# Stanford-ILIAD/PantheonRL

Hardware: AMD Instinct MI355X
Metric: env-steps/sec (all agents) Overcooked-simple PPO self-play (higher is better)
Workload: dtype f32; 1 GPU; OvercookedMultiEnv-v0 layout=simple, PPO self-play (two independent PPO learners per GPU), synthetic (n_envs, n_steps, obs_dim) rollouts; n_envs=1024, n_steps=128, obs_dim=62, features=62, n_logits=6, batch_size=32768, n_epochs=10, agents_per_gpu=2, parallelism=2 agent(s) per gpu x1 gpu(s) = 2 learners (single process), launch_mode=graph, gemm_mode=2, action_masks=none, rollout=scripted, rollout_requested=scripted

## Files before the change

pantheonrl_amd/csrc/ph_policy.hip:

```cpp
#include <cstring>
#include <initializer_list>
#include "ph_rowtail.h"
#include "ph_liar_group.h"
#include "ph_pool.h"

namespace ph {


template <int R, int LP, bool VALU>
__device__ __forceinline__ void policy_fwd_body(const FwdArgs& a) {
  extern __shared__ __attribute__((aligned(16))) float smem[];
  constexpr int NT = R * 4;
  const NetDims& nd = a.nd;
  constexpr int Lp = LP, LDO = LP + 1;
  float* bufA = smem;
  float* bufB = bufA + R * LDH;
  float* w1s = bufB + R * LDH;
  float* w2s = w1s + HID * LDH;
  float* wos = w2s + HID * LDH;
  float* outs = wos + HID * LDO;
  float* b1s = outs + R * LDO;
  float* b2s = b1s + HID;
  float* bos = b2s + HID;
  int* rowphys = (int*)(bos + 64);
// ... 120 lines not shown
    return (i == 5 && (tid >> 6) != 1) ? NONE : base + (unsigned)(3 * i) * (unsigned)D * 4u;
  }
  __device__ __forceinline__ static __amdgpu_buffer_rsrc_t block(const float* blk, int n, int D) {
    return __builtin_amdgcn_make_buffer_rsrc(const_cast<float*>(blk), 0, n * D * 4, 0x00020000);
  }
  __device__ __forceinline__ void issue(const float* obs, int n, const NetDims& nd, unsigned base, int tid) {
    const __amdgpu_buffer_rsrc_t rs = block(obs, n, nd.D);
#pragma unroll
    for (int i = 0; i < ITERS; ++i)
      v[i] = __builtin_bit_cast(float, __builtin_amdgcn_raw_buffer_load_b32(rs, slot_offset(base, i, nd.D, tid), 0, 0));
  }
  __device__ __forceinline__ void commit(float* dst, int tid) const {
    const int kk = tid & 63, w = (tid >> 6) - 1;
#pragma unroll
    for (int i = 0; i < ITERS; ++i) {
      const int r = w + 3 * i;
      if (r < 16) dst[r * LDH + kk] = v[i];
    }
  }
  __device__ __forceinline__ void copy_out(float* rb_obs, int n, int D, unsigned base, int tid) const {
    const __amdgpu_buffer_rsrc_t rs = block(rb_obs, n, D);
#pragma unroll
    for (int i = 0; i < ITERS; ++i)
      __builtin_amdgcn_raw_buffer_store_b32(__builtin_bit_cast(unsigned, v[i]), rs, slot_offset(base, i, D, tid), 0, 0);
  }
};

template <int CTRL>
__device__ __forceinline__ float dpp_quad_f(float v) {
  return __builtin_bit_cast(float, __builtin_amdgcn_update_dpp(0, __builtin_bit_cast(int, v), CTRL, 0xF, 0xF, true));
}
__device__ __forceinline__ float quad_sum_f(float v) {
  v += dpp_quad_f<0xB1>(v);
  v += dpp_quad_f<0x4E>(v);
  return v;
}

template <bool KEEP_JOINT>
__device__ __forceinline__ void fwd_args_pin_lean(FwdArgs& a) {
  a.mask = nullptr;
  a.uniforms = nullptr;
  a.given_actions = nullptr;
  a.deterministic = 0;
  a.act_f32 = nullptr;
  a.entropy = nullptr;
  a.logits = nullptr;
#ifndef PH_LEAN_PROF
  a.prof = nullptr;
#endif
  a.pos_env = nullptr;
  a.rec_mask = nullptr;
  if constexpr (!KEEP_JOINT) {
    a.joint = nullptr;
    a.joint_ll = nullptr;
  }
  a.env_mask = nullptr;
  a.host_done = nullptr;
  __builtin_assume(a.rb_obs != nullptr);
  __builtin_assume(a.rb_act != nullptr);
  __builtin_assume(a.rb_rew != nullptr);
  __builtin_assume(a.rb_es != nullptr);
  __builtin_assume(a.rb_val != nullptr);
  __builtin_assume(a.rb_logp != nullptr);
  __builtin_assume(a.es_in != nullptr);
}
bool fwd_args_lean(const FwdArgs& a, bool joint_ok = false) {
  static int enabled = -1;
  if (enabled < 0) {
    const char* e = getenv("PH_ROLLOUT_LEAN");
    enabled = (e && e[0] == '0') ? 0 : 1;
  }
#ifdef PH_LEAN_PROF
  constexpr bool lean_prof = true;
#else
  constexpr bool lean_prof = false;
#endif
  return enabled && !a.mask && !a.uniforms && !a.given_actions && !a.deterministic && !a.act_f32 && !a.entropy && !a.logits && (lean_prof || !a.prof) &&
         !a.pos_env && !a.rec_mask && (joint_ok || (!a.joint && !a.joint_ll)) && !a.env_mask && !a.host_done && a.rb_obs && a.rb_act && a.rb_rew &&
         a.rb_es && a.rb_val && a.rb_logp && a.es_in;
}

constexpr int ZS_FLOATS = 4 * 16 * 8;

template <bool VALU, int LEAN = 0>
__device__ __forceinline__ void policy_fwd16_body(const FwdArgs& a0, const ph_p2p* px = nullptr, int px_t = 0, int px_a_local = 0,
                                                  int agent = 0, const ScriptedSteps* sc = nullptr, int px_persistent = 0) {
  extern __shared__ __attribute__((aligned(16))) float smem[];
  constexpr int R = 16, NT = 256;
  const NetDims& nd = a0.nd;
  FwdArgs a = a0;
  if constexpr (LEAN == 1) fwd_args_pin_lean<false>(a);
  if constexpr (LEAN == 2) fwd_args_pin_lean<true>(a);
#ifdef PH_LEAN_PROF
  long long* const prof0 = a0.prof;
#else
  long long* const prof0 = LEAN ? nullptr : a0.prof;
#endif
  float* xs = smem;
  float* hs = xs + R * LDH;
  float* zs = hs + R * LDH;
  int* rowphys = (int*)(zs + ZS_FLOATS);
  float* upre = (float*)(rowphys + 16);
  unsigned long long** pxll = (unsigned long long**)(upre + 32);

  const int tid = threadIdx.x;
  const int wave = tid >> 6, lane = tid & 63, c = lane & 15, g = lane >> 4;
  const int net = blockIdx.y;
  const int row0 = blockIdx.x * R;
  const ph_layout& lay = nd.lay;
  const float* W1 = a.params + (net == 0 ? lay.pi_W1 : lay.vf_W1);
  const float* B1 = a.params + (net == 0 ? lay.pi_b1 : lay.vf_b1);
  const float* W2 = a.params + (net == 0 ? lay.pi_W2 : lay.vf_W2);
  const float* B2 = a.params + (net == 0 ? lay.pi_b2 : lay.vf_b2);
  const int nk = nd.L;

  PH_STAMP(a.prof, 0);
  if (tid < R) rowphys[tid] = (row0 + tid < a.n) ? row0 + tid : -1;
  constexpr bool PXH = LEAN != 0;
  const int pxw_h = (PXH && px) ? px->world : 0, pxc_h = (PXH && px) ? px->count : 0, pxr_h = (PXH && px) ? px->rank : 0;
  const int pxT_h = (PXH && px) ? px->T : 1, pxslots_h = (PXH && px) ? px->ll_slots : 1;
  unsigned long long* const ll_self_h = (PXH && px) ? px->ll[pxr_h] : nullptr;
  if (PXH && px && tid < pxw_h && tid < PH_MAX_RANKS) pxll[tid] = px->ll[tid];
#define pxw (PXH ? pxw_h : px->world)
#define pxc (PXH ? pxc_h : px->count)
#define pxr (PXH ? pxr_h : px->rank)
#define pxT (PXH ? pxT_h : px->T)
#define pxslots (PXH ? pxslots_h : px->ll_slots)
#define ll_self (PXH ? ll_self_h : px->ll[px->rank])
#define PXLL(p) (PXH ? pxll[p] : px->ll[p])
  float bw1[16], bw2[16], bwh[4];
  const int col = 16 * wave + c;
#pragma unroll
  for (int s = 0; s < 16; ++s) {
    const int k = g + 4 * s;
    bw1[s] = (k < nd.F) ? W1[k * HID + col] : 0.f;
    bw2[s] = W2[k * HID + col];
  }
#pragma unroll
  for (int s = 0; s < 4; ++s) {
    const int k = g + 4 * (4 * wave + s);
    bwh[s] = 0.f;
    if (net == 0) {
      if (c < nk) bwh[s] = a.params[lay.act_W + k * nk + c];
    } else if (c == 0) {
      bwh[s] = a.params[lay.val_W + k];
    }
  }
  const float bias1 = B1[col], bias2 = B2[col];
  float hbias = 0.f;
  if (wave == 0) {
    if (net == 0) hbias = (c < nk) ? a.params[lay.act_b + c] : 0.f;
    else hbias = (c == 0) ? a.params[lay.val_b] : 0.f;
  }
  XStage<R, NT> xr;
  lds_only_barrier();
  if (sc) a.obs = sc->obs_seq;
  xr.issue(rowphys, a.obs, nd, 0);
  const bool staged = sc != nullptr && nd.obs_kind == PH_SPACE_BOX;
  const bool copy_staged = staged && net == 1 && a.rb_obs && !a.pos_env && wave != 0;
  const unsigned roff = RowStage3::base_offset(row0, nd, tid);
  RowStage3 rows;
  if (copy_staged) rows.issue(a.obs, a0.n, nd, roff, tid);
  xr.commit(xs, rowphys, a.obs, nd, 0);
  vm_drain();
  if (copy_staged) rows.copy_out(a.rb_obs, a0.n, nd.D, roff, tid);
  lds_only_barrier();
  PH_STAMP(a.prof, 1);

  const int n_steps = sc ? sc->n_steps : 1;
  unsigned long long epoch_hi = 0ull;
  if (sc) {
    epoch_hi = a0.epoch ? (unsigned long long)(*a0.epoch) << 32 : 0ull;
    a.epoch = nullptr;
    a.counter = a0.counter + epoch_hi;
  }
  const unsigned long long px_epoch = (px && px_persistent) ? *px->epoch : 0ull;
  const bool draw_ahead = sc && net == 0 && !a.uniforms && !a.deterministic && !a.given_actions;
  auto draw_uniforms = [&](int t1) {
    if (lane < R && row0 + lane < a0.n)
      upre[(t1 & 1) * R + lane] = philox_uniform(a0.seed, a0.counter + (unsigned long long)t1 + epoch_hi, (uint32_t)(row0 + lane), 0u);
  };
  if (draw_ahead && wave == 1) draw_uniforms(0);

  auto product = [&](const float* A, const float (&bw)[16]) -> f32x4 {
    f32x4 e = {0.f, 0.f, 0.f, 0.f}, o = {0.f, 0.f, 0.f, 0.f};
    const float* ap = A + c * LDH + g;
    float av[16];
#pragma unroll
    for (int s = 0; s < 16; ++s) av[s] = ap[4 * s];
    __builtin_amdgcn_sched_barrier(0);
#pragma unroll
    for (int s = 0; s < 16; s += 2) {
      e = mma16<VALU>(av[s], bw[s], e, lane);
      o = mma16<VALU>(av[s + 1], bw[s + 1], o, lane);
    }
    return e + o;
  };

  for (int t = 0; t < n_steps; ++t) {
  long long* const pstep = (sc && t == 8) ? prof0 : nullptr;
  PH_STAMP(pstep, 8);
  if (t > 0) {
    const size_t row = (size_t)t * a0.n;
    a.obs = sc->obs_seq + row * nd.D;
    a.counter = a0.counter + (unsigned long long)t + epoch_hi;
    a.rb_obs = a0.rb_obs + row * nd.D;
    a.rb_act = a0.rb_act + row * nd.A;
    a.rb_rew = a0.rb_rew + row;
    a.rb_es = a0.rb_es + row;
    a.rb_val = a0.rb_val + row;
    a.rb_logp = a0.rb_logp + row;
    a.es_in = sc->done_seq + (row - a0.n);
    a.pending_reward = sc->rew_seq + (row - a0.n);
    a.prev_rew = a0.rb_rew + (row - a0.n);
    if constexpr (!LEAN) {
      a.mask = (sc->mask_seq && sc->mask_policy) ? sc->mask_seq + row * nd.L : nullptr;
      a.env_mask = (sc->mask_seq && sc->mask_env) ? sc->mask_seq + row * nd.L : nullptr;
    }
    if (px_persistent && a0.joint) {
      a.joint = a0.joint;
      a.joint_ll = ll_self + (size_t)p2p_persistent_slot(px_epoch, pxT, t - 1) * pxw * pxc;
      a.ll_t = t - 1;
    }
    a.prof = nullptr;
    if (!staged) {
      xr.issue(rowphys, a.obs, nd, 0);
      xr.commit(xs, rowphys, a.obs, nd, 0);
      vm_drain();
    }
    lds_only_barrier();
  }
  PH_STAMP(pstep, 9);
  const bool more = t + 1 < n_steps;
  const float* const obs_next = sc ? sc->obs_seq + (size_t)(t + 1) * a0.n * nd.D : nullptr;

  const bool pre_ok = net == 1 && wave == 0 && lane < R && row0 + lane < a.n && !a.pos_env && a.rb_val;
  ValuePre vpre = {0.f, 0.f, 0.f, 0ull, 0ull, 0u, 0, 0};
  if (pre_ok) vpre = value_row_preload(a, row0 + lane);
  const bool copy_from_regs = net == 1 && a.rb_obs && !a.pos_env && nd.obs_kind == PH_SPACE_BOX;
  {
    const f32x4 z1 = product(xs, bw1);
#pragma unroll
    for (int r = 0; r < 4; ++r) hs[(4 * g + r) * LDH + col] = fast_tanh(z1[r] + bias1);
  }
  lds_only_barrier();
  PH_STAMP(a.prof, 3);
  PH_STAMP(pstep, 10);
  {
    const f32x4 z2 = product(hs, bw2);
#pragma unroll
    for (int r = 0; r < 4; ++r) xs[(4 * g + r) * LDH + col] = fast_tanh(z2[r] + bias2);
  }
  lds_only_barrier();
  PH_STAMP(a.prof, 5);
  PH_STAMP(pstep, 11);

  if (staged && net == 1 && more && wave != 0) rows.issue(obs_next, a0.n, nd, roff, tid);

  {
    if (wave == 0 && pre_ok) value_row_preload_words(a, row0 + lane, vpre);
    const float* ap = xs + c * LDH + g + 16 * wave;
    float av[4];
#pragma unroll
    for (int j = 0; j < 4; ++j) av[j] = ap[4 * j];
    f32x4 e = {0.f, 0.f, 0.f, 0.f}, o = {0.f, 0.f, 0.f, 0.f};
    e = mma16<VALU>(av[0], bwh[0], e, lane);
    o = mma16<VALU>(av[1], bwh[1], o, lane);
    e = mma16<VALU>(av[2], bwh[2], e, lane);
    o = mma16<VALU>(av[3], bwh[3], o, lane);
    const f32x4 zh = e + o;
    if (c < 8) {
#pragma unroll
      for (int r = 0; r < 4; ++r) zs[(wave * R + 4 * g + r) * 8 + c] = zh[r] + hbias;
    }
  }
  lds_only_barrier();
  PH_STAMP(pstep, 12);
  if (sc) vm_drain();
  if (staged && more && wave != 0) {
    if (net == 1) {
      rows.commit(xs, tid);
      if (copy_staged) rows.copy_out(a0.rb_obs + (size_t)(t + 1) * a0.n * nd.D, a0.n, nd.D, roff, tid);
    }
  }
  if (wave == 0) {
    PH_STAMP(pstep, 13);
    const int r = lane, grow = row0 + lane;
    if (r < R && grow < a.n) {
      float z[8];
      {
        float4 q[4][2];
#pragma unroll
        for (int w = 0; w < 4; ++w) {
          q[w][0] = *reinterpret_cast<const float4*>(zs + (w * R + r) * 8);
          q[w][1] = *reinterpret_cast<const float4*>(zs + (w * R + r) * 8 + 4);
        }
#pragma unroll
        for (int h = 0; h < 2; ++h) {
          z[4 * h + 0] = (q[0][h].x + q[1][h].x) + (q[2][h].x + q[3][h].x);
          z[4 * h + 1] = (q[0][h].y + q[1][h].y) + (q[2][h].y + q[3][h].y);
          z[4 * h + 2] = (q[0][h].z + q[1][h].z) + (q[2][h].z + q[3][h].z);
          z[4 * h + 3] = (q[0][h].w + q[1][h].w) + (q[2][h].w + q[3][h].w);
        }
      }
      if (net == 0) {
        const float* up = draw_ahead ? upre + (t & 1) * R + r : nullptr;
        const uint64_t ctr = fwd_counter(a);
        int act;
        switch (nk) {
          case 1: act = discrete8_row_tail<1>(a, nd, grow, z, ctr, up, pstep); break;
          case 2: act = discrete8_row_tail<2>(a, nd, grow, z, ctr, up, pstep); break;
          case 3: act = discrete8_row_tail<3>(a, nd, grow, z, ctr, up, pstep); break;
          case 4: act = discrete8_row_tail<4>(a, nd, grow, z, ctr, up, pstep); break;
          case 5: act = discrete8_row_tail<5>(a, nd, grow, z, ctr, up, pstep); break;
          case 6: act = discrete8_row_tail<6>(a, nd, grow, z, ctr, up, pstep); break;
          case 7: act = discrete8_row_tail<7>(a, nd, grow, z, ctr, up, pstep); break;
          default: act = discrete8_row_tail<8>(a, nd, grow, z, ctr, up, pstep); break;
        }
        if (px) {
          const int pt = px_t + t;
          const int slot = px_persistent ? p2p_persistent_slot(px_epoch, pxT, pt) : pt % pxslots;
          const size_t off = (size_t)slot * pxw * pxc + (size_t)(pxr * px_a_local + agent) * a.n + grow;
          const unsigned long long w =
              ((unsigned long long)p2p_stamp32(px_persistent ? px_epoch : *px->epoch, pxT, pt) << 32) | (unsigned long long)(unsigned)act;
          for (int p = 0; p < pxw; ++p)
            __hip_atomic_store(PXLL(p) + off, w, __ATOMIC_RELAXED, __HIP_MEMORY_SCOPE_SYSTEM);
        }
      } else {
        value_row_tail(a, grow, z[0], !a.pos_env && a.rb_val, vpre);
        if (sc && t == n_steps - 1) {
          float add = sc->rew_seq[(size_t)t * a0.n + grow];
          if (px_persistent && a0.joint) {
            FwdArgs b = a;
            b.joint_ll = ll_self + (size_t)p2p_persistent_slot(px_epoch, pxT, t) * pxw * pxc;
            b.ll_t = t;
            int p = *a0.partner_seat;
            p = p < 0 ? 0 : (p >= a0.n_seats ? a0.n_seats - 1 : p);
            const int mine = ll_read(b, b.joint_ll + (size_t)a0.seat * a0.n + grow);
            const int theirs = ll_read(b, b.joint_ll + (size_t)p * a0.n + grow);
            add += joint_reward(mine, theirs, a0.bonus, a0.reward_rule);
          }
          a.rb_rew[grow] += add;
        }
      }
    }
  }
  PH_STAMP(pstep, 14);
  const bool stage_here = staged && net == 0 && more && wave != 0;
  if (stage_here) rows.issue(obs_next, a0.n, nd, roff, tid);
  if (draw_ahead && wave == 1 && more) draw_uniforms(t + 1);
  if (stage_here) {
    rows.commit(xs, tid);
    vm_drain();
  }
  if (copy_from_regs) {
    if (!staged) {
      const int kk = tid & 63;
#pragma unroll
      for (int i = 0; i < XStage<R, NT>::ITERS; ++i) {
        const int rr = (tid + NT * i) >> 6;
        if (kk < nd.D && row0 + rr < a.n) a.rb_obs[(size_t)(row0 + rr) * nd.D + kk] = xr.v[i];
      }
    }
  } else if (net == 1) {
    copy_obs_rows(a, row0, (a.n - row0 < R) ? a.n - row0 : R, nd.D);
  }
  PH_STAMP(a.prof, 7);
  PH_STAMP(pstep, 15);
  }
}

#undef pxw
#undef pxc
#undef pxr
#undef pxT
#undef pxslots
#undef ll_self
#undef PXLL

template <bool VALU, bool LEAN = false>
__global__ __launch_bounds__(256) void policy_fwd16_kernel(FwdArgs a) {
  policy_fwd16_body<VALU, LEAN ? 1 : 0>(a);
  if constexpr (!LEAN) {
    if (a.host_done) {
      __threadfence_system();
      __syncthreads();
      if (threadIdx.x == 0) __hip_atomic_store(a.host_done + blockIdx.y, a.host_seq, __ATOMIC_RELEASE, __HIP_MEMORY_SCOPE_SYSTEM);
    }
  }
}
template <bool VALU, bool LEAN>
__global__ __launch_bounds__(256) void policy_fwd16_rollout_kernel(FwdArgs a, ScriptedSteps sc) {
  policy_fwd16_body<VALU, LEAN ? 1 : 0>(a, nullptr, 0, 0, 0, &sc);
}
template <bool LEAN>
__global__ __launch_bounds__(256) void policy_fwd16_multi_kernel(FwdMulti m) {
  policy_fwd16_body<false, LEAN ? 2 : 0>(m.a[blockIdx.z], m.px.x, m.px.t, m.px.a_local, blockIdx.z);
}
template <bool LEAN>
__global__ __launch_bounds__(256, 3) void policy_fwd16_exchange_rollout_kernel(FwdMulti m, ScriptedMulti sm) {
  policy_fwd16_body<false, LEAN ? 2 : 0>(m.a[blockIdx.z], m.px.x, 0, m.px.a_local, blockIdx.z, &sm.sc[blockIdx.z], 1);
}

static size_t fwd16_lds_bytes() { return sizeof(float) * (size_t)(2 * 16 * LDH + ZS_FLOATS + 16 + 32) + sizeof(void*) * PH_MAX_RANKS; }

bool fwd16_eligible(const NetDims& nd, int n) {
  static int enabled = -1;
  if (enabled < 0) {
    const char* e = getenv("PH_FWD16");
    enabled = (e && e[0] == '0') ? 0 : 1;
  }
  return enabled && !nd.gauss && nd.nchunk == 1 && nd.A == 1 && nd.L <= 8 && n < 16384;
}

template <bool VALU>
static hipError_t launch_fwd16_variant(const FwdArgs& a, hipStream_t s) {
  const size_t lds = fwd16_lds_bytes();
  const bool general = VALU || !fwd_args_lean(a);
  const void* fn = general ? (const void*)policy_fwd16_kernel<VALU> : (const void*)policy_fwd16_kernel<false, true>;
  if (const hipError_t e = allow_dynamic_lds(fn, lds); e != hipSuccess) return e;
  if (general) hipLaunchKernelGGL((policy_fwd16_kernel<VALU>), dim3((a.n + 15) / 16, 2), dim3(256), lds, s, a);
  else hipLaunchKernelGGL((policy_fwd16_kernel<false, true>), dim3((a.n + 15) / 16, 2), dim3(256), lds, s, a);
  return hipGetLastError();
}

static size_t rollout_lds_bytes(int nwg_total) {
  const int cu = device_cu_count();
  return (cu > 0 && 2 * nwg_total <= cu) ? (size_t)81 * 1024 + 512 : fwd16_lds_bytes();
}
hipError_t launch_policy_fwd16_rollout(const FwdArgs& a, const ScriptedSteps& sc, int gemm_mode, hipStream_t s) {
  dim3 grid((a.n + 15) / 16, 2), block(256);
  const size_t lds = rollout_lds_bytes((int)(grid.x * grid.y));
  const int variant = gemm_mode == 1 ? 1 : ((fwd_args_lean(a) && !sc.mask_seq) ? 2 : 0);
  const void* fn = variant == 1 ? (const void*)policy_fwd16_rollout_kernel<true, false>
                                : (variant == 2 ? (const void*)policy_fwd16_rollout_kernel<false, true> : (const void*)policy_fwd16_rollout_kernel<false, false>);
  if (const hipError_t e = allow_dynamic_lds(fn, lds); e != hipSuccess) return e;
  if (variant == 1) hipLaunchKernelGGL((policy_fwd16_rollout_kernel<true, false>), grid, block, lds, s, a, sc);
  else if (variant == 2) hipLaunchKernelGGL((policy_fwd16_rollout_kernel<false, true>), grid, block, lds, s, a, sc);
  else hipLaunchKernelGGL((policy_fwd16_rollout_kernel<false, false>), grid, block, lds, s, a, sc);
  return hipGetLastError();
}

hipError_t exchange_rollout_blocks_per_cu(int* blocks_out) {
  const size_t lds = fwd16_lds_bytes();
  int api = 0;
  hipError_t e = hipOccupancyMaxActiveBlocksPerMultiprocessor(&api, (const void*)policy_fwd16_exchange_rollout_kernel<false>, 256, lds);
  if (e != hipSuccess) return e;
  const int by_lds = (int)((size_t)160 * 1024 / lds);
  int blocks = api < 8 ? api : 8;
  if (blocks > by_lds) blocks = by_lds;
  else if (blocks < by_lds && blocks > 1) blocks -= 1;
  *blocks_out = blocks < 1 ? 1 : blocks;
  return hipSuccess;
}

hipError_t launch_policy_fwd16_exchange_rollout(const FwdMulti& m, const ScriptedMulti& sm, int n_agents, hipStream_t s) {
  bool lean = true;
  for (int i = 0; i < n_agents; ++i) lean = lean && fwd_args_lean(m.a[i], true) && !sm.sc[i].mask_seq;
  const dim3 grid((m.a[0].n + 15) / 16, 2, n_agents);
  if (lean) hipLaunchKernelGGL(policy_fwd16_exchange_rollout_kernel<true>, grid, dim3(256), fwd16_lds_bytes(), s, m, sm);
  else hipLaunchKernelGGL(policy_fwd16_exchange_rollout_kernel<false>, grid, dim3(256), fwd16_lds_bytes(), s, m, sm);
  return hipGetLastError();
}

template <int CTRL>
__device__ __forceinline__ float dpp_f(float v) {
  return __builtin_bit_cast(float, __builtin_amdgcn_update_dpp(0, __builtin_bit_cast(int, v), CTRL, 0xF, 0xF, true));
}
template <bool MAX>
__device__ __forceinline__ float seg_scan32(float v, int k, int lo) {
  const int kr = k & 15;
#define PH_SCAN_STEP(D, CTRL)                                   \
  {                                                             \
    const float o = dpp_f<CTRL>(v);                             \
    const bool ok = kr >= (D) && k - (D) >= lo;                 \
    v = ok ? (MAX ? fmaxf(v, o) : v + o) : v;                   \
  }
  PH_SCAN_STEP(1, 0x111)
  PH_SCAN_STEP(2, 0x112)
  PH_SCAN_STEP(4, 0x114)
  PH_SCAN_STEP(8, 0x118)
#undef PH_SCAN_STEP
  const float o = dpp_f<0x142>(v);
  const bool ok = k >= 16 && lo <= 15;
  return ok ? (MAX ? fmaxf(v, o) : v + o) : v;
}
__device__ __forceinline__ float sum32_upper(float v) {
  v += dpp_f<0xB1>(v);
  v += dpp_f<0x4E>(v);
  v += dpp_f<0x124>(v);
  v += dpp_f<0x128>(v);
  return v + dpp_f<0x142>(v);
}
__device__ __forceinline__ bool head_draws(const FwdArgs& a) { return !a.given_actions && !a.deterministic && !a.uniforms; }
__device__ __forceinline__ float head_draw32(const FwdArgs& a, int g, bool row_ok, int comp, uint64_t ctr) {
  return (row_ok && comp >= 0) ? philox_uniform(a.seed, ctr, (uint32_t)g, (uint32_t)comp) : 0.f;
}
__device__ __forceinline__ void head_tail32(const FwdArgs& a, const NetDims& nd, int g, bool row_ok, long long ridx, float z,
                                            int k, int lo, int last, int comp, float u_drawn) {
  const bool own = row_ok && comp >= 0;
  const int nk = last - lo + 1;
  if (own && a.mask) z = z - 30.0f * (1.0f - (float)(a.mask[(size_t)g * nd.L + k] != 0));
  if (own && a.logits) a.logits[(size_t)g * nd.L + k] = z;
  const float M = __shfl(seg_scan32<true>(z, k, lo), last, 32);
  const float e = fast_exp(z - M);
  const float s = seg_scan32<false>(e, k, lo);
  const float S = __shfl(s, last, 32);
  const float lse = M + fast_log(S), inv = __builtin_amdgcn_rcpf(S);
  const int half = (threadIdx.x >> 5) & 1;
  int act = 0;
  if (a.given_actions) {
    act = own ? (int)a.given_actions[(size_t)g * nd.A + comp] : 0;
    act = act < 0 ? 0 : (act >= nk ? nk - 1 : act);
  } else if (a.deterministic) {
    const unsigned long long b = __ballot(z == M);
    const unsigned bits = ((unsigned)(b >> (32 * half)) >> lo) & (nk >= 32 ? 0xffffffffu : ((1u << nk) - 1u));
// ... 1006 lines not shown
```

pantheonrl_amd/csrc/ph_rowtail.h:

```cpp
#pragma once
#include "ph_launch.h"

namespace ph {

__device__ __forceinline__ long long rb_row(const FwdArgs& a, int g) {
  if (!a.pos_env) return g;
  const int p = a.pos_env[g];
  if (!a.rec_mask[g] || p >= a.rb_T) return -1;
  return (long long)p * a.n + g;
}

__device__ __forceinline__ int ll_read(const FwdArgs& a, const unsigned long long* word) {
  const unsigned want = p2p_stamp32(*a.ll_epoch, a.ll_T, a.ll_t);
  const long long t0 = wall_clock64();
  int polls = 0;
  while (true) {
    const unsigned long long v = __hip_atomic_load(word, __ATOMIC_RELAXED, __HIP_MEMORY_SCOPE_SYSTEM);
    if ((unsigned)(v >> 32) == want) return (int)(unsigned)v;
    if ((unsigned long long)(wall_clock64() - t0) > a.ll_timeout) {
      p2p_note_timeout(a.ll_error, 1, a.ll_t, a.joint_ll ? (unsigned long long)(word - a.joint_ll) : 0ull, want, v);
      return (int)(unsigned)v;
    }
    poll_backoff(polls);
  }
// ... 29 lines not shown
  ValuePre p;
  p.es = a.es_in ? a.es_in[g] : 0.f;
  p.pend = a.pending_reward ? a.pending_reward[g] : 0.f;
  p.prev = (a.pending_reward && a.prev_rew) ? a.prev_rew[g] : 0.f;
  p.w_mine = p.w_theirs = 0ull;
  p.want = 0u;
  p.partner = 0;
  p.has_words = 0;
  return p;
}

__device__ __forceinline__ void value_row_preload_words(const FwdArgs& a, int g, ValuePre& p) {
  if (a.pending_reward && a.joint && a.joint_ll) {
    int q = *a.partner_seat;
    q = q < 0 ? 0 : (q >= a.n_seats ? a.n_seats - 1 : q);
    p.partner = q;
    p.want = p2p_stamp32(*a.ll_epoch, a.ll_T, a.ll_t);
    p.w_mine = __hip_atomic_load(a.joint_ll + (size_t)a.seat * a.n + g, __ATOMIC_RELAXED, __HIP_MEMORY_SCOPE_SYSTEM);
    p.w_theirs = __hip_atomic_load(a.joint_ll + (size_t)q * a.n + g, __ATOMIC_RELAXED, __HIP_MEMORY_SCOPE_SYSTEM);
    p.has_words = 1;
  }
}

__device__ __forceinline__ void value_row_tail(const FwdArgs& a, int g, float v, bool has_pre = false,
                                               ValuePre pre = ValuePre{0.f, 0.f, 0.f, 0ull, 0ull, 0u, 0, 0}) {
  const long long ridx = a.rb_val ? rb_row(a, g) : -1;
  if (a.values && (!a.pos_env || ridx >= 0)) a.values[g] = v;
  if (ridx >= 0) {
    a.rb_val[ridx] = v;
    a.rb_rew[ridx] = 0.f;
    a.rb_es[ridx] = has_pre ? pre.es : a.es_in[g];
    if (a.pending_reward) {
      float add = has_pre ? pre.pend : a.pending_reward[g];
      if (a.joint) {
        int p = *a.partner_seat;
        p = p < 0 ? 0 : (p >= a.n_seats ? a.n_seats - 1 : p);
        if (a.joint_ll) {
          int mine, theirs;
          if (has_pre && pre.has_words && pre.partner == p && (unsigned)(pre.w_mine >> 32) == pre.want &&
              (unsigned)(pre.w_theirs >> 32) == pre.want) {
            mine = (int)(unsigned)pre.w_mine;
            theirs = (int)(unsigned)pre.w_theirs;
          } else {
            ll_read2(a, a.joint_ll + (size_t)a.seat * a.n + g, a.joint_ll + (size_t)p * a.n + g, mine, theirs);
          }
          add += joint_reward(mine, theirs, a.bonus, a.reward_rule);
        } else {
          add += joint_reward(a.joint[(size_t)a.seat * a.n + g], a.joint[(size_t)p * a.n + g], a.bonus, a.reward_rule);
        }
      }
      if (has_pre) a.prev_rew[g] = pre.prev + add;
      else a.prev_rew[g] += add;
    }
  }
}

__device__ __forceinline__ void copy_obs_rows(const FwdArgs& a, int row0, int nrow, int D, int tid = -1, int nt = 0) {
  if (!a.rb_obs) return;
  if (tid < 0) {
    tid = threadIdx.x;
    nt = blockDim.x;
  }
  if (!a.pos_env) {
    const size_t off = (size_t)row0 * D;
    for (int e = tid; e < nrow * D; e += nt) a.rb_obs[off + e] = a.obs[off + e];
  } else {
    for (int e = tid; e < nrow * D; e += nt) {
      const int r = e / D, d = e - r * D;
      const long long ridx = rb_row(a, row0 + r);
      if (ridx >= 0) a.rb_obs[(size_t)ridx * D + d] = a.obs[(size_t)(row0 + r) * D + d];
    }
  }
}

__device__ __forceinline__ uint64_t fwd_counter(const FwdArgs& a) {
  return a.counter + (a.epoch ? (uint64_t)(*a.epoch) << 32 : 0ull);
}

#if defined(PH_TAIL_STAMPS)
#define PH_TAIL_STAMP(slot) PH_STAMP(tail_dbg, slot)
#else
#define PH_TAIL_STAMP(slot) do { } while (0)
#endif
template <int NK = 8>
__device__ __forceinline__ int discrete8_row_tail(const FwdArgs& a, const NetDims& nd, int g, float (&zr)[8], uint64_t ctr,
                                                  const float* u_pre = nullptr, long long* tail_dbg = nullptr) {
  const int nk = NK < 8 ? NK : nd.L;
  if (a.mask) {
#pragma unroll
    for (int k = 0; k < 8; ++k)
      if (k < nk) zr[k] = zr[k] - 30.0f * (1.0f - (float)(a.mask[(size_t)g * nk + k] != 0));
  }
  if (a.logits) {
#pragma unroll
    for (int k = 0; k < 8; ++k)
      if (k < nk) a.logits[(size_t)g * nk + k] = zr[k];
  }
  float pr[8];
  float m = -3.0e38f;
#pragma unroll
  for (int k = 0; k < 8; ++k) {
    if (NK < 8 && k >= NK) continue;
    zr[k] = (k < nk) ? zr[k] : -3.0e38f;
    m = fmaxf(m, zr[k]);
  }
  float se = 0.f;
#pragma unroll
  for (int k = 0; k < 8; ++k) {
    pr[k] = 0.f;
    if (NK < 8 && k >= NK) continue;
    pr[k] = (k < nk) ? fast_exp(zr[k] - m) : 0.f;
    se += pr[k];
  }
  const float lse = m + fast_log(se), inv = __builtin_amdgcn_rcpf(se);
  PH_TAIL_STAMP(2);
  int act = 0;
  if (a.given_actions) {
    act = (int)a.given_actions[g];
    act = act < 0 ? 0 : (act >= nk ? nk - 1 : act);
  } else if (a.deterministic) {
    float best = zr[0];
#pragma unroll
    for (int k = 1; k < 8; ++k)
      if (k < nk && zr[k] > best) { best = zr[k]; act = k; }
  } else {
    const float u = a.uniforms ? a.uniforms[g] : (u_pre ? *u_pre : philox_uniform(a.seed, ctr, (uint32_t)g, 0u));
    float cum = 0.f;
#pragma unroll
    for (int k = 0; k < 7; ++k) {
      if (NK < 8 && k >= NK - 1) continue;
      cum += pr[k] * inv;
      act += (k < nk - 1 && u >= cum) ? 1 : 0;
    }
  }
  PH_TAIL_STAMP(4);
  float zact = 0.f, ent = 0.f;
#pragma unroll
  for (int k = 0; k < 8; ++k) {
    if (NK < 8 && k >= NK) continue;
    const float lp = zr[k] - lse;
    ent -= (k < nk) ? pr[k] * inv * lp : 0.f;
    zact = (k == act) ? zr[k] : zact;
  }
  const float logp = zact - lse;
  int env_act = act;
  if (a.env_mask && a.env_mask[(size_t)g * nk + act] == 0) {
    env_act = 0;
#pragma unroll
    for (int k = 7; k >= 0; --k)
      if (k < nk && a.env_mask[(size_t)g * nk + k] != 0) env_act = k;
  }
  PH_TAIL_STAMP(6);
  if (a.act_i32) a.act_i32[g] = env_act;
  if (a.act_f32) a.act_f32[g] = (float)act;
  if (a.logp) a.logp[g] = logp;
  if (a.entropy) a.entropy[g] = ent;
  if (a.rb_act || a.rb_logp) {
    const long long ridx = rb_row(a, g);
    if (ridx >= 0) {
      if (a.rb_act) a.rb_act[ridx] = (float)act;
      if (a.rb_logp) a.rb_logp[ridx] = logp;
    }
  }
  return env_act;
}

__device__ __forceinline__ void general_row_tail(const FwdArgs& a, const NetDims& nd, int g, float* z, uint64_t ctr) {
  const bool small = !nd.gauss && nd.A == 1 && nd.L <= 8;
  if (a.mask && !small) {
    for (int k = 0; k < nd.L; ++k) z[k] = z[k] - 30.0f * (1.0f - (float)(a.mask[(size_t)g * nd.L + k] != 0));
  }
  if (a.logits && !small)
    for (int k = 0; k < nd.L; ++k) a.logits[(size_t)g * nd.L + k] = z[k];
  float logp = 0.f, ent = 0.f;
  if (nd.gauss) {
    const float* ls = a.params + nd.lay.val_b + 1;
    for (int c = 0; c < nd.A; ++c) {
      const float mu = z[c], lsd = ls[c];
      float act;
      if (a.given_actions) act = a.given_actions[(size_t)g * nd.A + c];
      else if (a.deterministic) act = mu;
      else {
        float eps;
        if (a.uniforms) eps = a.uniforms[(size_t)g * nd.A + c];
        else {
          const float u1 = philox_uniform(a.seed, ctr, (uint32_t)g, (uint32_t)c);
          const float u2 = philox_uniform(a.seed, ctr, (uint32_t)g, (uint32_t)(c + 128));
          eps = __builtin_sqrtf(-2.0f * fast_log(fmaxf(u1, 1.0e-30f))) * __builtin_cosf(6.28318530717958647692f * u2);
        }
        act = mu + fast_exp(lsd) * eps;
      }
      const float d = (act - mu) * fast_exp(-lsd);
      logp += (-0.5f * d * d - lsd) - 0.91893853320467274178f;
      ent += 1.41893853320467274178f + lsd;
      if (a.act_f32) a.act_f32[(size_t)g * nd.A + c] = act;
      if (a.rb_act) {
        const long long ridx = rb_row(a, g);
        if (ridx >= 0) a.rb_act[(size_t)ridx * nd.A + c] = act;
      }
    }
  } else if (small) {
    float zr[8];
#pragma unroll
    for (int k = 0; k < 8; ++k) zr[k] = (k < nd.L) ? z[k] : 0.f;
    discrete8_row_tail(a, nd, g, zr, fwd_counter(a));
    return;
  } else
  for (int c = 0; c < nd.A; ++c) {
    const int lo = nd.act_off[c], nk = nd.act_off[c + 1] - lo;
    float m = z[lo];
    for (int k = 1; k < nk; ++k) m = fmaxf(m, z[lo + k]);
    float se = 0.f;
    for (int k = 0; k < nk; ++k) se += fast_exp(z[lo + k] - m);
    const float lse = m + fast_log(se);
    int act;
    if (a.given_actions) {
      act = (int)a.given_actions[(size_t)g * nd.A + c];
      act = act < 0 ? 0 : (act >= nk ? nk - 1 : act);
    } else if (a.deterministic) {
      act = 0;
      float best = z[lo];
      for (int k = 1; k < nk; ++k)
        if (z[lo + k] > best) { best = z[lo + k]; act = k; }
    } else {
      const float u = a.uniforms ? a.uniforms[(size_t)g * nd.A + c]
                                 : philox_uniform(a.seed, ctr, (uint32_t)g, (uint32_t)c);
      float cum = 0.f;
      act = 0;
      for (int k = 0; k < nk - 1; ++k) {
        cum += fast_exp(z[lo + k] - lse);
        act += (u >= cum) ? 1 : 0;
      }
    }
    float e = 0.f;
    for (int k = 0; k < nk; ++k) {
// ... 22 lines not shown
```

Before: 115.6 million agent-steps/s.

## Add dedicated tail wave to overlap row sampling with next-step MLP compute

For the MFMA rollout path, the block grows from 256 to 320 threads and the fifth wave becomes a tail wave. It handles per-row softmax sampling, value write-back, uniform drawing and value preloads, while the four compute waves move on to the next step's GEMMs. The tail wave meets the compute waves through a fixed barrier schedule, and its split point releases them once the action and lse are known. Compute waves get raised priority, and obs staging is reorganised so all non-zero compute waves commit. This adds barrier-matching complexity and one extra wave per block, and the launcher now rejects masked, given-action and deterministic calls.

```diff
diff --git a/pantheonrl_amd/csrc/ph_policy.hip b/pantheonrl_amd/csrc/ph_policy.hip
--- a/pantheonrl_amd/csrc/ph_policy.hip
+++ b/pantheonrl_amd/csrc/ph_policy.hip
@@ -226,7 +226,18 @@
 
 constexpr int ZS_FLOATS = 4 * 16 * 8;
 
-template <bool VALU, int LEAN = 0>
+struct TailWaveHook {
+  bool arrive, alive;
+  long long* stamp;
+  __device__ __forceinline__ void split(int act, float lse) const {
+    if (stamp) stamp[4] = (long long)clock64();
+    if (arrive) asm volatile("s_waitcnt lgkmcnt(0)\n\ts_barrier" ::"v"(act), "v"(lse) : "memory");
+    else asm volatile("" ::"v"(act), "v"(lse));
+  }
+  __device__ __forceinline__ bool live() const { return alive; }
+};
+
+template <bool VALU, int LEAN = 0, int TW = 0>
 __device__ __forceinline__ void policy_fwd16_body(const FwdArgs& a0, const ph_p2p* px = nullptr, int px_t = 0, int px_a_local = 0,
                                                   int agent = 0, const ScriptedSteps* sc = nullptr, int px_persistent = 0) {
   extern __shared__ __attribute__((aligned(16))) float smem[];
@@ -235,6 +246,13 @@
   FwdArgs a = a0;
   if constexpr (LEAN == 1) fwd_args_pin_lean<false>(a);
   if constexpr (LEAN == 2) fwd_args_pin_lean<true>(a);
+  if constexpr (TW != 0) {
+    a.mask = nullptr;
+    a.env_mask = nullptr;
+    a.uniforms = nullptr;
+    a.given_actions = nullptr;
+    a.deterministic = 0;
+  }
 #ifdef PH_LEAN_PROF
   long long* const prof0 = a0.prof;
 #else
@@ -248,7 +266,8 @@
   unsigned long long** pxll = (unsigned long long**)(upre + 32);
 
   const int tid = threadIdx.x;
-  const int wave = tid >> 6, lane = tid & 63, c = lane & 15, g = lane >> 4;
+  const int wave = TW ? __builtin_amdgcn_readfirstlane(tid >> 6) : tid >> 6, lane = tid & 63, c = lane & 15, g = lane >> 4;
+  const bool lw = TW == 0 || wave < 4;
   const int net = blockIdx.y;
   const int row0 = blockIdx.x * R;
   const ph_layout& lay = nd.lay;
@@ -277,20 +296,21 @@
 #pragma unroll
   for (int s = 0; s < 16; ++s) {
     const int k = g + 4 * s;
-    bw1[s] = (k < nd.F) ? W1[k * HID + col] : 0.f;
-    bw2[s] = W2[k * HID + col];
+    bw1[s] = (lw && k < nd.F) ? W1[k * HID + col] : 0.f;
+    bw2[s] = lw ? W2[k * HID + col] : 0.f;
   }
 #pragma unroll
   for (int s = 0; s < 4; ++s) {
     const int k = g + 4 * (4 * wave + s);
     bwh[s] = 0.f;
+    if (!lw) continue;
     if (net == 0) {
       if (c < nk) bwh[s] = a.params[lay.act_W + k * nk + c];
     } else if (c == 0) {
       bwh[s] = a.params[lay.val_W + k];
     }
   }
-  const float bias1 = B1[col], bias2 = B2[col];
+  const float bias1 = lw ? B1[col] : 0.f, bias2 = lw ? B2[col] : 0.f;
   float hbias = 0.f;
   if (wave == 0) {
     if (net == 0) hbias = (c < nk) ? a.params[lay.act_b + c] : 0.f;
@@ -299,13 +319,15 @@
   XStage<R, NT> xr;
   lds_only_barrier();
   if (sc) a.obs = sc->obs_seq;
-  xr.issue(rowphys, a.obs, nd, 0);
+  const bool xsync = nd.obs_kind != PH_SPACE_BOX;
+  if (lw) xr.issue(rowphys, a.obs, nd, 0);
   const bool staged = sc != nullptr && nd.obs_kind == PH_SPACE_BOX;
-  const bool copy_staged = staged && net == 1 && a.rb_obs && !a.pos_env && wave != 0;
+  const bool copy_staged = staged && net == 1 && a.rb_obs && !a.pos_env && (TW ? wave != 0 && wave < 4 : wave != 0);
   const unsigned roff = RowStage3::base_offset(row0, nd, tid);
   RowStage3 rows;
   if (copy_staged) rows.issue(a.obs, a0.n, nd, roff, tid);
-  xr.commit(xs, rowphys, a.obs, nd, 0);
+  if (lw) xr.commit(xs, rowphys, a.obs, nd, 0);
+  if (TW != 0 && !lw && xsync) lds_only_barrier();
   vm_drain();
   if (copy_staged) rows.copy_out(a.rb_obs, a0.n, nd.D, roff, tid);
   lds_only_barrier();
@@ -324,7 +346,7 @@
     if (lane < R && row0 + lane < a0.n)
       upre[(t1 & 1) * R + lane] = philox_uniform(a0.seed, a0.counter + (unsigned long long)t1 + epoch_hi, (uint32_t)(row0 + lane), 0u);
   };
-  if (draw_ahead && wave == 1) draw_uniforms(0);
+  if (TW == 0 && draw_ahead && wave == 1) draw_uniforms(0);
 
   auto product = [&](const float* A, const float (&bw)[16]) -> f32x4 {
     f32x4 e = {0.f, 0.f, 0.f, 0.f}, o = {0.f, 0.f, 0.f, 0.f};
@@ -341,10 +363,7 @@
     return e + o;
   };
 
-  for (int t = 0; t < n_steps; ++t) {
-  long long* const pstep = (sc && t == 8) ? prof0 : nullptr;
-  PH_STAMP(pstep, 8);
-  if (t > 0) {
+  auto step_record = [&](FwdArgs& a, int t) {
     const size_t row = (size_t)t * a0.n;
     a.obs = sc->obs_seq + row * nd.D;
     a.counter = a0.counter + (unsigned long long)t + epoch_hi;
@@ -357,7 +376,7 @@
     a.es_in = sc->done_seq + (row - a0.n);
     a.pending_reward = sc->rew_seq + (row - a0.n);
     a.prev_rew = a0.rb_rew + (row - a0.n);
-    if constexpr (!LEAN) {
+    if constexpr (!LEAN && TW == 0) {
       a.mask = (sc->mask_seq && sc->mask_policy) ? sc->mask_seq + row * nd.L : nullptr;
       a.env_mask = (sc->mask_seq && sc->mask_env) ? sc->mask_seq + row * nd.L : nullptr;
     }
@@ -367,110 +386,49 @@
       a.ll_t = t - 1;
     }
     a.prof = nullptr;
-    if (!staged) {
-      xr.issue(rowphys, a.obs, nd, 0);
-      xr.commit(xs, rowphys, a.obs, nd, 0);
-      vm_drain();
-    }
-    lds_only_barrier();
-  }
-  PH_STAMP(pstep, 9);
-  const bool more = t + 1 < n_steps;
-  const float* const obs_next = sc ? sc->obs_seq + (size_t)(t + 1) * a0.n * nd.D : nullptr;
-
-  const bool pre_ok = net == 1 && wave == 0 && lane < R && row0 + lane < a.n && !a.pos_env && a.rb_val;
-  ValuePre vpre = {0.f, 0.f, 0.f, 0ull, 0ull, 0u, 0, 0};
-  if (pre_ok) vpre = value_row_preload(a, row0 + lane);
-  const bool copy_from_regs = net == 1 && a.rb_obs && !a.pos_env && nd.obs_kind == PH_SPACE_BOX;
-  {
-    const f32x4 z1 = product(xs, bw1);
-#pragma unroll
-    for (int r = 0; r < 4; ++r) hs[(4 * g + r) * LDH + col] = fast_tanh(z1[r] + bias1);
-  }
-  lds_only_barrier();
-  PH_STAMP(a.prof, 3);
-  PH_STAMP(pstep, 10);
-  {
-    const f32x4 z2 = product(hs, bw2);
-#pragma unroll
-    for (int r = 0; r < 4; ++r) xs[(4 * g + r) * LDH + col] = fast_tanh(z2[r] + bias2);
-  }
-  lds_only_barrier();
-  PH_STAMP(a.prof, 5);
-  PH_STAMP(pstep, 11);
-
-  if (staged && net == 1 && more && wave != 0) rows.issue(obs_next, a0.n, nd, roff, tid);
-
-  {
-    if (wave == 0 && pre_ok) value_row_preload_words(a, row0 + lane, vpre);
-    const float* ap = xs + c * LDH + g + 16 * wave;
-    float av[4];
-#pragma unroll
-    for (int j = 0; j < 4; ++j) av[j] = ap[4 * j];
-    f32x4 e = {0.f, 0.f, 0.f, 0.f}, o = {0.f, 0.f, 0.f, 0.f};
-    e = mma16<VALU>(av[0], bwh[0], e, lane);
-    o = mma16<VALU>(av[1], bwh[1], o, lane);
-    e = mma16<VALU>(av[2], bwh[2], e, lane);
-    o = mma16<VALU>(av[3], bwh[3], o, lane);
-    const f32x4 zh = e + o;
-    if (c < 8) {
-#pragma unroll
-      for (int r = 0; r < 4; ++r) zs[(wave * R + 4 * g + r) * 8 + c] = zh[r] + hbias;
-    }
-  }
-  lds_only_barrier();
-  PH_STAMP(pstep, 12);
-  if (sc) vm_drain();
-  if (staged && more && wave != 0) {
-    if (net == 1) {
-      rows.commit(xs, tid);
-      if (copy_staged) rows.copy_out(a0.rb_obs + (size_t)(t + 1) * a0.n * nd.D, a0.n, nd.D, roff, tid);
-    }
-  }
-  if (wave == 0) {
-    PH_STAMP(pstep, 13);
-    const int r = lane, grow = row0 + lane;
-    if (r < R && grow < a.n) {
-      float z[8];
-      {
-        float4 q[4][2];
-#pragma unroll
-        for (int w = 0; w < 4; ++w) {
-          q[w][0] = *reinterpret_cast<const float4*>(zs + (w * R + r) * 8);
-          q[w][1] = *reinterpret_cast<const float4*>(zs + (w * R + r) * 8 + 4);
-        }
-#pragma unroll
-        for (int h = 0; h < 2; ++h) {
-          z[4 * h + 0] = (q[0][h].x + q[1][h].x) + (q[2][h].x + q[3][h].x);
-          z[4 * h + 1] = (q[0][h].y + q[1][h].y) + (q[2][h].y + q[3][h].y);
-          z[4 * h + 2] = (q[0][h].z + q[1][h].z) + (q[2][h].z + q[3][h].z);
-          z[4 * h + 3] = (q[0][h].w + q[1][h].w) + (q[2][h].w + q[3][h].w);
-        }
-      }
-      if (net == 0) {
-        const float* up = draw_ahead ? upre + (t & 1) * R + r : nullptr;
-        const uint64_t ctr = fwd_counter(a);
-        int act;
-        switch (nk) {
-          case 1: act = discrete8_row_tail<1>(a, nd, grow, z, ctr, up, pstep); break;
-          case 2: act = discrete8_row_tail<2>(a, nd, grow, z, ctr, up, pstep); break;
-          case 3: act = discrete8_row_tail<3>(a, nd, grow, z, ctr, up, pstep); break;
-          case 4: act = discrete8_row_tail<4>(a, nd, grow, z, ctr, up, pstep); break;
-          case 5: act = discrete8_row_tail<5>(a, nd, grow, z, ctr, up, pstep); break;
-          case 6: act = discrete8_row_tail<6>(a, nd, grow, z, ctr, up, pstep); break;
-          case 7: act = discrete8_row_tail<7>(a, nd, grow, z, ctr, up, pstep); break;
-          default: act = discrete8_row_tail<8>(a, nd, grow, z, ctr, up, pstep); break;
-        }
-        if (px) {
-          const int pt = px_t + t;
-          const int slot = px_persistent ? p2p_persistent_slot(px_epoch, pxT, pt) : pt % pxslots;
-          const size_t off = (size_t)slot * pxw * pxc + (size_t)(pxr * px_a_local + agent) * a.n + grow;
-          const unsigned long long w =
-              ((unsigned long long)p2p_stamp32(px_persistent ? px_epoch : *px->epoch, pxT, pt) << 32) | (unsigned long long)(unsigned)act;
-          for (int p = 0; p < pxw; ++p)
-            __hip_atomic_store(PXLL(p) + off, w, __ATOMIC_RELAXED, __HIP_MEMORY_SCOPE_SYSTEM);
-        }
-      } else {
+  };
+
+  auto row_tail = [&](const FwdArgs& a, int t, int r, int grow, const ValuePre& vpre, const float* up, long long* pstep, auto hook) {
+    float z[8];
+    {
+      float4 q[4][2];
+#pragma unroll
+      for (int w = 0; w < 4; ++w) {
+        q[w][0] = *reinterpret_cast<const float4*>(zs + (w * R + r) * 8);
+        q[w][1] = *reinterpret_cast<const float4*>(zs + (w * R + r) * 8 + 4);
+      }
+#pragma unroll
+      for (int h = 0; h < 2; ++h) {
+        z[4 * h + 0] = (q[0][h].x + q[1][h].x) + (q[2][h].x + q[3][h].x);
+        z[4 * h + 1] = (q[0][h].y + q[1][h].y) + (q[2][h].y + q[3][h].y);
+        z[4 * h + 2] = (q[0][h].z + q[1][h].z) + (q[2][h].z + q[3][h].z);
+        z[4 * h + 3] = (q[0][h].w + q[1][h].w) + (q[2][h].w + q[3][h].w);
+      }
+    }
+    if (net == 0) {
+      const uint64_t ctr = fwd_counter(a);
+      int act;
+      switch (nk) {
+        case 1: act = discrete8_row_tail<1>(a, nd, grow, z, ctr, up, pstep, hook); break;
+        case 2: act = discrete8_row_tail<2>(a, nd, grow, z, ctr, up, pstep, hook); break;
+        case 3: act = discrete8_row_tail<3>(a, nd, grow, z, ctr, up, pstep, hook); break;
+        case 4: act = discrete8_row_tail<4>(a, nd, grow, z, ctr, up, pstep, hook); break;
+        case 5: act = discrete8_row_tail<5>(a, nd, grow, z, ctr, up, pstep, hook); break;
+        case 6: act = discrete8_row_tail<6>(a, nd, grow, z, ctr, up, pstep, hook); break;
+        case 7: act = discrete8_row_tail<7>(a, nd, grow, z, ctr, up, pstep, hook); break;
+        default: act = discrete8_row_tail<8>(a, nd, grow, z, ctr, up, pstep, hook); break;
+      }
+      if (px && hook.live()) {
+        const int pt = px_t + t;
+        const int slot = px_persistent ? p2p_persistent_slot(px_epoch, pxT, pt) : pt % pxslots;
+        const size_t off = (size_t)slot * pxw * pxc + (size_t)(pxr * px_a_local + agent) * a.n + grow;
+        const unsigned long long w =
+            ((unsigned long long)p2p_stamp32(px_persistent ? px_epoch : *px->epoch, pxT, pt) << 32) | (unsigned long long)(unsigned)act;
+        for (int p = 0; p < pxw; ++p)
+          __hip_atomic_store(PXLL(p) + off, w, __ATOMIC_RELAXED, __HIP_MEMORY_SCOPE_SYSTEM);
+      }
+    } else {
+      if (hook.live()) {
         value_row_tail(a, grow, z[0], !a.pos_env && a.rb_val, vpre);
         if (sc && t == n_steps - 1) {
           float add = sc->rew_seq[(size_t)t * a0.n + grow];
@@ -487,12 +445,128 @@
           a.rb_rew[grow] += add;
         }
       }
-    }
+      hook.split(0, z[0]);
+    }
+  };
+
+  if constexpr (TW != 0) {
+    if (!lw) {
+      const int nlive = (a0.n - row0 < R) ? a0.n - row0 : R;
+      const int r = lane < nlive ? lane : nlive - 1, grow = row0 + r;
+      const bool live = lane < nlive;
+#ifdef PH_LEAN_PROF
+      long long* const wstamp = (prof0 && lane == 0) ? prof0 + ((size_t)blockIdx.y * gridDim.x + blockIdx.x) * 16 : nullptr;
+#else
+      long long* const wstamp = nullptr;
+#endif
+      auto draw = [&](int t) { return philox_uniform(a0.seed, a0.counter + (unsigned long long)t + epoch_hi, (uint32_t)grow, 0u); };
+      auto preload = [&](const FwdArgs& a) {
+        return (net == 1 && !a.pos_env && a.rb_val) ? value_row_preload(a, grow) : ValuePre{0.f, 0.f, 0.f, 0ull, 0ull, 0u, 0, 0};
+      };
+      if (draw_ahead) upre[r] = draw(0);
+      ValuePre vpre = preload(a);
+      lds_only_barrier();
+      lds_only_barrier();
+      lds_only_barrier();
+      for (int s = 0; s < n_steps; ++s) {
+        const bool more = s + 1 < n_steps;
+        if (more) {
+          if (xsync) lds_only_barrier();
+          lds_only_barrier();
+        }
+        long long* const ws = (s == 7) ? wstamp : nullptr;
+        if (ws) ws[2] = (long long)clock64();
+        row_tail(a, s, r, grow, vpre, draw_ahead ? upre + r : nullptr, nullptr, TailWaveHook{more, live, ws});
+        if (ws) ws[6] = (long long)clock64();
+        if (more) {
+          step_record(a, s + 1);
+          vpre = preload(a);
+          lds_only_barrier();
+          if (draw_ahead) upre[r] = draw(s + 1);
+          lds_only_barrier();
+        }
+      }
+      return;
+    }
+    __builtin_amdgcn_s_setprio(1);
+  }
+
+  for (int t = 0; t < n_steps; ++t) {
+  long long* const pstep = (sc && t == 8) ? prof0 : nullptr;
+  PH_STAMP(pstep, 8);
+  if (t > 0) {
+    step_record(a, t);
+    if (!staged) {
+      xr.issue(rowphys, a.obs, nd, 0);
+      xr.commit(xs, rowphys, a.obs, nd, 0);
+      vm_drain();
+    }
+    lds_only_barrier();
+  }
+  PH_STAMP(pstep, 9);
+  const bool more = t + 1 < n_steps;
+  const float* const obs_next = sc ? sc->obs_seq + (size_t)(t + 1) * a0.n * nd.D : nullptr;
+  if (TW != 0 && staged && more && wave != 0) rows.issue(obs_next, a0.n, nd, roff, tid);
+
+  const bool pre_ok = TW == 0 && net == 1 && wave == 0 && lane < R && row0 + lane < a.n && !a.pos_env && a.rb_val;
+  ValuePre vpre = {0.f, 0.f, 0.f, 0ull, 0ull, 0u, 0, 0};
+  if (pre_ok) vpre = value_row_preload(a, row0 + lane);
+  const bool copy_from_regs = net == 1 && a.rb_obs && !a.pos_env && nd.obs_kind == PH_SPACE_BOX;
+  {
+    const f32x4 z1 = product(xs, bw1);
+#pragma unroll
+    for (int r = 0; r < 4; ++r) hs[(4 * g + r) * LDH + col] = fast_tanh(z1[r] + bias1);
+  }
+  lds_only_barrier();
+  PH_STAMP(a.prof, 3);
+  PH_STAMP(pstep, 10);
+  {
+    const f32x4 z2 = product(hs, bw2);
+#pragma unroll
+    for (int r = 0; r < 4; ++r) xs[(4 * g + r) * LDH + col] = fast_tanh(z2[r] + bias2);
+  }
+  lds_only_barrier();
+  PH_STAMP(a.prof, 5);
+  PH_STAMP(pstep, 11);
+
+  if (TW == 0 && staged && net == 1 && more && wave != 0) rows.issue(obs_next, a0.n, nd, roff, tid);
+
+  {
+    if (wave == 0 && pre_ok) value_row_preload_words(a, row0 + lane, vpre);
+    const float* ap = xs + c * LDH + g + 16 * wave;
+    float av[4];
+#pragma unroll
+    for (int j = 0; j < 4; ++j) av[j] = ap[4 * j];
+    f32x4 e = {0.f, 0.f, 0.f, 0.f}, o = {0.f, 0.f, 0.f, 0.f};
+    e = mma16<VALU>(av[0], bwh[0], e, lane);
+    o = mma16<VALU>(av[1], bwh[1], o, lane);
+    e = mma16<VALU>(av[2], bwh[2], e, lane);
+    o = mma16<VALU>(av[3], bwh[3], o, lane);
+    const f32x4 zh = e + o;
+    if (c < 8) {
+#pragma unroll
+      for (int r = 0; r < 4; ++r) zs[(wave * R + 4 * g + r) * 8 + c] = zh[r] + hbias;
+    }
+  }
+  lds_only_barrier();
+  PH_STAMP(pstep, 12);
+  if (sc) vm_drain();
+  if (staged && more && wave != 0 && lw) {
+    if (net == 1 || TW != 0) {
+      rows.commit(xs, tid);
+      if (copy_staged) rows.copy_out(a0.rb_obs + (size_t)(t + 1) * a0.n * nd.D, a0.n, nd.D, roff, tid);
+    }
+  }
+  if (TW != 0) PH_STAMP(pstep, 13);
+  if (TW == 0 && wave == 0) {
+    PH_STAMP(pstep, 13);
+    const int r = lane, grow = row0 + lane;
+    if (r < R && grow < a.n) row_tail(a, t, r, grow, vpre, draw_ahead ? upre + (t & 1) * R + r : nullptr, pstep, TailNoHook{});
   }
   PH_STAMP(pstep, 14);
-  const bool stage_here = staged && net == 0 && more && wave != 0;
+  const bool stage_here = TW == 0 && staged && net == 0 && more && wave != 0;
   if (stage_here) rows.issue(obs_next, a0.n, nd, roff, tid);
-  if (draw_ahead && wave == 1 && more) draw_uniforms(t + 1);
+  if (TW == 0 && draw_ahead && wave == 1 && more) draw_uniforms(t + 1);
   if (stage_here) {
     rows.commit(xs, tid);
     vm_drain();
@@ -507,7 +581,7 @@
       }
     }
   } else if (net == 1) {
-    copy_obs_rows(a, row0, (a.n - row0 < R) ? a.n - row0 : R, nd.D);
+    copy_obs_rows(a, row0, (a.n - row0 < R) ? a.n - row0 : R, nd.D, TW ? tid : -1, NT);
   }
   PH_STAMP(a.prof, 7);
   PH_STAMP(pstep, 15);
@@ -533,9 +607,10 @@
     }
   }
 }
+constexpr int ROLLOUT_THREADS = 320;
 template <bool VALU, bool LEAN>
-__global__ __launch_bounds__(256) void policy_fwd16_rollout_kernel(FwdArgs a, ScriptedSteps sc) {
-  policy_fwd16_body<VALU, LEAN ? 1 : 0>(a, nullptr, 0, 0, 0, &sc);
+__global__ __launch_bounds__(VALU ? 256 : ROLLOUT_THREADS) void policy_fwd16_rollout_kernel(FwdArgs a, ScriptedSteps sc) {
+  policy_fwd16_body<VALU, LEAN ? 1 : 0, VALU ? 0 : 4>(a, nullptr, 0, 0, 0, &sc);
 }
 template <bool LEAN>
 __global__ __launch_bounds__(256) void policy_fwd16_multi_kernel(FwdMulti m) {
@@ -573,9 +648,10 @@
   return (cu > 0 && 2 * nwg_total <= cu) ? (size_t)81 * 1024 + 512 : fwd16_lds_bytes();
 }
 hipError_t launch_policy_fwd16_rollout(const FwdArgs& a, const ScriptedSteps& sc, int gemm_mode, hipStream_t s) {
-  dim3 grid((a.n + 15) / 16, 2), block(256);
+  if (a.mask || a.env_mask || a.uniforms || a.given_actions || a.deterministic || sc.mask_seq) return hipErrorInvalidValue;
+  const int variant = gemm_mode == 1 ? 1 : (fwd_args_lean(a) ? 2 : 0);
+  dim3 grid((a.n + 15) / 16, 2), block(variant == 1 ? 256 : ROLLOUT_THREADS);
   const size_t lds = rollout_lds_bytes((int)(grid.x * grid.y));
-  const int variant = gemm_mode == 1 ? 1 : ((fwd_args_lean(a) && !sc.mask_seq) ? 2 : 0);
   const void* fn = variant == 1 ? (const void*)policy_fwd16_rollout_kernel<true, false>
                                 : (variant == 2 ? (const void*)policy_fwd16_rollout_kernel<false, true> : (const void*)policy_fwd16_rollout_kernel<false, false>);
   if (const hipError_t e = allow_dynamic_lds(fn, lds); e != hipSuccess) return e;
diff --git a/pantheonrl_amd/csrc/ph_rowtail.h b/pantheonrl_amd/csrc/ph_rowtail.h
--- a/pantheonrl_amd/csrc/ph_rowtail.h
+++ b/pantheonrl_amd/csrc/ph_rowtail.h
@@ -135,16 +135,20 @@
 #else
 #define PH_TAIL_STAMP(slot) do { } while (0)
 #endif
-template <int NK = 8>
+struct TailNoHook {
+  __device__ __forceinline__ void split(int, float) const {}
+  __device__ __forceinline__ constexpr bool live() const { return true; }
+};
+template <int NK = 8, class Hook = TailNoHook>
 __device__ __forceinline__ int discrete8_row_tail(const FwdArgs& a, const NetDims& nd, int g, float (&zr)[8], uint64_t ctr,
-                                                  const float* u_pre = nullptr, long long* tail_dbg = nullptr) {
+                                                  const float* u_pre = nullptr, long long* tail_dbg = nullptr, const Hook hook = Hook{}) {
   const int nk = NK < 8 ? NK : nd.L;
   if (a.mask) {
 #pragma unroll
     for (int k = 0; k < 8; ++k)
       if (k < nk) zr[k] = zr[k] - 30.0f * (1.0f - (float)(a.mask[(size_t)g * nk + k] != 0));
   }
-  if (a.logits) {
+  if (a.logits && hook.live()) {
 #pragma unroll
     for (int k = 0; k < 8; ++k)
       if (k < nk) a.logits[(size_t)g * nk + k] = zr[k];
@@ -187,6 +191,7 @@
     }
   }
   PH_TAIL_STAMP(4);
+  hook.split(act, lse);
   float zact = 0.f, ent = 0.f;
 #pragma unroll
   for (int k = 0; k < 8; ++k) {
@@ -204,6 +209,7 @@
       if (k < nk && a.env_mask[(size_t)g * nk + k] != 0) env_act = k;
   }
   PH_TAIL_STAMP(6);
+  if (!hook.live()) return env_act;
   if (a.act_i32) a.act_i32[g] = env_act;
   if (a.act_f32) a.act_f32[g] = (float)act;
   if (a.logp) a.logp[g] = logp;
```

New measurement: 119.2 million agent-steps/s (median of 6 runs). 1.03x the previous value.
